# Hxyz-123/GoMatching

Hardware: AMD Instinct MI355X
Metric: frames/sec (whole node), 1280x720 clip, 100 queries/frame (higher is better)
Workload: dtype f32 (f16x3 split MFMA: 22-bit significand products, fp32 accumulate; parity tests at fp32 tolerances)

## Files before the change

gomatching_amd/csrc/msda.hip:

```cpp
#include <mutex>
#include <type_traits>
#include <vector>

#include "common.h"

namespace {

constexpr int HEADS = 8, CH = 32, LEVELS = 4;

__device__ __forceinline__ long xcd_contiguous_block(unsigned bid, unsigned nwg) {
    const unsigned q = nwg >> 3, r = nwg & 7, xcd = bid & 7;
    return (long)(xcd < r ? xcd * (q + 1) : r * (q + 1) + (xcd - r) * q) + (bid >> 3);
}

template <int POINTS>
__global__ __launch_bounds__(256) void msda_fwd_kernel(const float* __restrict__ value,
                                                       const int64_t* __restrict__ shapes,
                                                       const int64_t* __restrict__ lsi,
                                                       const float* __restrict__ loc,
                                                       const float* __restrict__ attw, float* __restrict__ out,
                                                       int B, int Lq, long v_bs, int v_rs) {
    const long q_global = xcd_contiguous_block(blockIdx.x, gridDim.x) * 4 + (threadIdx.x >> 6);
    if (q_global >= (long)B * Lq) return;
    const int lane = threadIdx.x & 63;
// ... 248 lines not shown
    const __amdgpu_buffer_rsrc_t rs = gom_buffer_rsrc(value + (size_t)b * v_bs, 0x7FFFFFFF);
    const unsigned mine = (unsigned)k * 16u;
    f32x4 acc = {0.f, 0.f, 0.f, 0.f};
#pragma unroll
    for (int i = 0; i < LP; ++i) {
        const int o = i >> 1, t = i & 1;
        const unsigned a1 = __builtin_bit_cast(unsigned, group8_read(__builtin_bit_cast(float, so1[t]), o)) + mine;
        const unsigned a2 = __builtin_bit_cast(unsigned, group8_read(__builtin_bit_cast(float, so2[t]), o)) + mine;
        const unsigned a3 = __builtin_bit_cast(unsigned, group8_read(__builtin_bit_cast(float, so3[t]), o)) + mine;
        const unsigned a4 = __builtin_bit_cast(unsigned, group8_read(__builtin_bit_cast(float, so4[t]), o)) + mine;
        const f32x4 v1 = __builtin_bit_cast(f32x4, __builtin_amdgcn_raw_buffer_load_b128(rs, (int)a1, 0, 0));
        const f32x4 v2 = __builtin_bit_cast(f32x4, __builtin_amdgcn_raw_buffer_load_b128(rs, (int)a2, 0, 0));
        const f32x4 v3 = __builtin_bit_cast(f32x4, __builtin_amdgcn_raw_buffer_load_b128(rs, (int)a3, 0, 0));
        const f32x4 v4 = __builtin_bit_cast(f32x4, __builtin_amdgcn_raw_buffer_load_b128(rs, (int)a4, 0, 0));
        const float w1 = group8_read(sw1[t], o), w2 = group8_read(sw2[t], o), w3 = group8_read(sw3[t], o), w4 = group8_read(sw4[t], o);
        msda_fma4(acc, w1, v1);
        msda_fma4(acc, w2, v2);
        msda_fma4(acc, w3, v3);
        msda_fma4(acc, w4, v4);
    }
    *reinterpret_cast<f32x4*>(out + (size_t)q_global * (HEADS * CH) + m * CH + k * 4) = acc;
}

template <int TY, int TX, int R, int CAP, int NB, int GLV = 0>
__global__ __launch_bounds__(256, 2) void msda_window_kernel(const float* __restrict__ value,
                                                             const int64_t* __restrict__ shapes,
                                                             const int64_t* __restrict__ lsi,
                                                             const float* __restrict__ raw, int ld_raw,
                                                             const float* __restrict__ ref, float* __restrict__ out,
                                                             int Lq, long v_bs, int v_rs, int tiles_y, int tiles_x, int ql,
                                                             unsigned* __restrict__ slow_groups) {
    constexpr int POINTS = 4, LP = LEVELS * POINTS, ITERS = (TY * TX) / 32;
    extern __shared__ __attribute__((aligned(16))) unsigned char win[];
    const int tid = threadIdx.x, lane = tid & 63;
    const int wave = __builtin_amdgcn_readfirstlane(tid >> 6);
    const int g = lane >> 3, k = lane & 7;
    const int m = (int)(blockIdx.x & 7u);
    unsigned tile = blockIdx.x >> 3;
    const int tx = (int)(tile % (unsigned)tiles_x);
    tile /= (unsigned)tiles_x;
    const int ty = (int)(tile % (unsigned)tiles_y);
    const int b = (int)(tile / (unsigned)tiles_y);
    const int l = k >> 1;

    int Hs[LEVELS], Ws[LEVELS];
    unsigned lv[LEVELS];
#pragma unroll
    for (int i = 0; i < LEVELS; ++i) {
        Hs[i] = (int)shapes[2 * i];
        Ws[i] = (int)shapes[2 * i + 1];
        lv[i] = (unsigned)lsi[i];
    }
    const int Hq = ql == 0 ? Hs[0] : ql == 1 ? Hs[1] : ql == 2 ? Hs[2] : Hs[3];
    const int Wq = ql == 0 ? Ws[0] : ql == 1 ? Ws[1] : ql == 2 ? Ws[2] : Ws[3];
    const long q0 = (long)b * Lq + (long)(ql == 0 ? lv[0] : ql == 1 ? lv[1] : ql == 2 ? lv[2] : lv[3]);
    const int y0t = ty * TY, x0t = tx * TX;
    const int y1t = min(y0t + TY, Hq) - 1, x1t = min(x0t + TX, Wq) - 1;
    const long qa = q0 + (long)y0t * Wq + x0t, qz = q0 + (long)y1t * Wq + x1t;
    const float rxa = ref[qa * 2], rya = ref[qa * 2 + 1], rxz = ref[qz * 2], ryz = ref[qz * 2 + 1];
    int wx0[LEVELS], wy0[LEVELS], wx1[LEVELS], wy1[LEVELS], wwd[LEVELS];
#pragma unroll
    for (int i = 0; i < LEVELS; ++i) {
        int ax = (int)floorf(fminf(rxa, rxz) * Ws[i] - 0.5f) - R, zx = (int)floorf(fmaxf(rxa, rxz) * Ws[i] - 0.5f) + R + 1;
        int ay = (int)floorf(fminf(rya, ryz) * Hs[i] - 0.5f) - R, zy = (int)floorf(fmaxf(rya, ryz) * Hs[i] - 0.5f) + R + 1;
        ax = max(ax, 0); ay = max(ay, 0); zx = min(zx, Ws[i] - 1); zy = min(zy, Hs[i] - 1);
        if (zx < ax) zx = ax;
        if (zy < ay) zy = ay;
        int w_ = zx - ax + 1, h_ = zy - ay + 1;
        if (w_ > CAP) { w_ = CAP; zx = ax + w_ - 1; }
        if (w_ * h_ > CAP) { h_ = CAP / w_; zy = ay + h_ - 1; }
        wx0[i] = ax; wy0[i] = ay; wx1[i] = zx; wy1[i] = zy; wwd[i] = w_;
    }
    const int H = l == 0 ? Hs[0] : l == 1 ? Hs[1] : l == 2 ? Hs[2] : Hs[3];
    const int W = l == 0 ? Ws[0] : l == 1 ? Ws[1] : l == 2 ? Ws[2] : Ws[3];
    const int mx0 = l == 0 ? wx0[0] : l == 1 ? wx0[1] : l == 2 ? wx0[2] : wx0[3];
    const int my0 = l == 0 ? wy0[0] : l == 1 ? wy0[1] : l == 2 ? wy0[2] : wy0[3];
    const int mx1 = l == 0 ? wx1[0] : l == 1 ? wx1[1] : l == 2 ? wx1[2] : wx1[3];
    const int my1 = l == 0 ? wy1[0] : l == 1 ? wy1[1] : l == 2 ? wy1[2] : wy1[3];
    const int mww = l == 0 ? wwd[0] : l == 1 ? wwd[1] : l == 2 ? wwd[2] : wwd[3];
    const unsigned lvl = l == 0 ? lv[0] : l == 1 ? lv[1] : l == 2 ? lv[2] : lv[3];
    const float Hf = (float)H, Wf = (float)W;
    const float rW = 1.f / Wf, rH = 1.f / Hf;

    const __amdgpu_buffer_rsrc_t rs = gom_buffer_rsrc(value + (size_t)b * v_bs, 0x7FFFFFFF);
    const unsigned mine = (unsigned)k * 16u;
    const unsigned head = (unsigned)(m * CH) * 4u;

    float sw1[ITERS][2], sw2[ITERS][2], sw3[ITERS][2], sw4[ITERS][2];
    unsigned pk[ITERS][2];
    unsigned go1[GLV ? ITERS : 1][2], go2[GLV ? ITERS : 1][2], go3[GLV ? ITERS : 1][2], go4[GLV ? ITERS : 1][2];
    f32x4 acc[ITERS];
    long qrow[ITERS];
    bool fast[ITERS], live[ITERS];
    f32x4 offs[ITERS];
    float lga[ITERS], lgb[ITERS], rxs[ITERS], rys[ITERS];
#pragma unroll
    for (int it = 0; it < ITERS; ++it) {
        const int j = (wave * ITERS + it) * 8 + g;
        const int jy = j / TX, jx = j - jy * TX;
        const int qy = y0t + jy, qx = x0t + jx;
        live[it] = qy <= y1t && qx <= x1t;
        const long q_global = q0 + (long)(live[it] ? qy : y0t) * Wq + (live[it] ? qx : x0t);
        qrow[it] = q_global;
        const float* op = raw + (size_t)q_global * ld_raw + m * (LP * 2) + 4 * k;
        const float* lp = raw + (size_t)q_global * ld_raw + HEADS * LP * 2 + m * LP + 2 * k;
        offs[it] = *reinterpret_cast<const f32x4*>(op);
        lga[it] = lp[0];
        lgb[it] = lp[1];
        rxs[it] = ref[q_global * 2];
        rys[it] = ref[q_global * 2 + 1];
    }
#define MSDA_GEOMETRY(IT, T, OFF4, RX, RY, E, INV_SUM, OK, SO)                                                    \
    {                                                                                                             \
        const float ox = (OFF4)[2 * (T)], oy = (OFF4)[2 * (T) + 1];                                               \
        float qx_ = ox * rW, qy_ = oy * rH;                                                                       \
        qx_ = fmaf(fmaf(-qx_, Wf, ox), rW, qx_);                                                                  \
        qy_ = fmaf(fmaf(-qy_, Hf, oy), rH, qy_);                                                                  \
        const float lx = (RX) + qx_, ly = (RY) + qy_;                                                             \
        const float w = (E) * (INV_SUM);                                                                          \
        const float h_im = ly * H - 0.5f, w_im = lx * W - 0.5f;                                                   \
        const bool inside = h_im > -1.f && w_im > -1.f && h_im < Hf && w_im < Wf;                                 \
        const float hf = floorf(h_im), wf = floorf(w_im);                                                         \
        const float lh = h_im - hf, lw = w_im - wf;                                                               \
        const float hh = 1.f - lh, hw = 1.f - lw;                                                                 \
        const int h_low = inside ? (int)hf : 0, w_low = inside ? (int)wf : 0;                                     \
        const bool y0 = h_low >= 0, y1 = h_low + 1 <= H - 1;                                                      \
        const bool x0 = w_low >= 0, x1 = w_low + 1 <= W - 1;                                                      \
        const int yc0 = y0 ? h_low : 0, yc1 = y1 ? h_low + 1 : H - 1;                                             \
        const int xc0 = x0 ? w_low : 0, xc1 = x1 ? w_low + 1 : W - 1;                                             \
        const unsigned r0 = lvl + (unsigned)(yc0 * W), r1 = lvl + (unsigned)(yc1 * W);                            \
        SO##1 = (r0 + xc0) * (unsigned)v_rs * 4u + head;                                                          \
        SO##2 = (r0 + xc1) * (unsigned)v_rs * 4u + head;                                                          \
        SO##3 = (r1 + xc0) * (unsigned)v_rs * 4u + head;                                                          \
        SO##4 = (r1 + xc1) * (unsigned)v_rs * 4u + head;                                                          \
        const float ww_ = inside ? w : 0.f;                                                                       \
        sw1[IT][T] = ((y0 && x0) ? hh * hw : 0.f) * ww_;                                                          \
        sw2[IT][T] = ((y0 && x1) ? hh * lw : 0.f) * ww_;                                                          \
        sw3[IT][T] = ((y1 && x0) ? lh * hw : 0.f) * ww_;                                                          \
        sw4[IT][T] = ((y1 && x1) ? lh * lw : 0.f) * ww_;                                                          \
         \
        OK = !inside || l < GLV || (yc0 >= my0 && yc1 <= my1 && xc0 >= mx0 && xc1 <= mx1);                        \
        const bool use = inside && OK;                          \
        const int ly0 = use ? yc0 - my0 : 0, lx0 = use ? xc0 - mx0 : 0;                                           \
        const unsigned la_ = (unsigned)((ly0 * mww + lx0) * 128);                                                 \
        pk[IT][T] = la_ | ((use && xc1 != xc0) ? (1u << 20) : 0u) | ((use && yc1 != yc0) ? (1u << 21) : 0u);      \
    }
    unsigned any_slow = 0;
#pragma unroll
    for (int it = 0; it < ITERS; ++it) {
        const float lg0 = lga[it], lg1 = lgb[it];
        float mx = fmaxf(lg0, lg1);
        mx = fmaxf(mx, __builtin_bit_cast(float, __builtin_amdgcn_ds_swizzle(__builtin_bit_cast(int, mx), 0x1F | (1 << 10))));
        mx = fmaxf(mx, __builtin_bit_cast(float, __builtin_amdgcn_ds_swizzle(__builtin_bit_cast(int, mx), 0x1F | (2 << 10))));
        mx = fmaxf(mx, __builtin_bit_cast(float, __builtin_amdgcn_ds_swizzle(__builtin_bit_cast(int, mx), 0x1F | (4 << 10))));
        const float e0 = expf(lg0 - mx), e1 = expf(lg1 - mx);
        float sum = 0.f;
#pragma unroll
        for (int o = 0; o < 8; ++o) {
            sum += group8_read(e0, o);
            sum += group8_read(e1, o);
        }
        const float inv_sum = 1.f / sum;
        bool ok0, ok1;
        unsigned sa1, sa2, sa3, sa4, sb1, sb2, sb3, sb4;
        MSDA_GEOMETRY(it, 0, offs[it], rxs[it], rys[it], e0, inv_sum, ok0, sa)
        MSDA_GEOMETRY(it, 1, offs[it], rxs[it], rys[it], e1, inv_sum, ok1, sb)
        if constexpr (GLV > 0) {
            go1[it][0] = sa1; go2[it][0] = sa2; go3[it][0] = sa3; go4[it][0] = sa4;
            go1[it][1] = sb1; go2[it][1] = sb2; go3[it][1] = sb3; go4[it][1] = sb4;
        }
        (void)sa1; (void)sa2; (void)sa3; (void)sa4; (void)sb1; (void)sb2; (void)sb3; (void)sb4;
        fast[it] = __builtin_amdgcn_ballot_w64(!(ok0 && ok1)) == 0;
        any_slow |= fast[it] ? 0u : 1u;
        acc[it] = f32x4{0.f, 0.f, 0.f, 0.f};
    }

    auto fill = [&](auto LEVC, unsigned char* buf) {
        constexpr int lev = decltype(LEVC)::value;
        const int ww_ = wwd[lev], n_lines = ww_ * (wy1[lev] - wy0[lev] + 1);
        const float inv_w = 1.f / (float)ww_;
        for (int base = wave * 8; base < n_lines; base += 32) {
            int line = base + g;
            if (line > n_lines - 1) line = n_lines - 1;
            int yy = (int)(((float)line + 0.5f) * inv_w);
            int xx = line - yy * ww_;
            if (xx < 0) { --yy; xx += ww_; }
            if (xx >= ww_) { ++yy; xx -= ww_; }
            const unsigned src = (lv[lev] + (unsigned)((wy0[lev] + yy) * Ws[lev] + wx0[lev] + xx)) * (unsigned)v_rs * 4u + head + mine;
            __builtin_amdgcn_raw_ptr_buffer_load_lds(rs, (__attribute__((address_space(3))) void*)(buf + (size_t)base * 128), 16,
                                                     (int)src, 0, 0, 0);
        }
    };
    auto bcast = [](float v, int owner) { return group8_read(v, owner); };
    auto level_samples = [&](auto LEVC, const unsigned char* buf) {
        constexpr int lev = decltype(LEVC)::value;
        typedef __attribute__((address_space(3))) f32x4 LdsF4;
        const unsigned mine_lds = mine + (unsigned)(size_t)buf;
        const unsigned row_bytes = (unsigned)wwd[lev] * 128u;
#pragma unroll
        for (int pnt = 0; pnt < POINTS; ++pnt) {
            const int i = lev * POINTS + pnt, o = i >> 1, t = i & 1;
#pragma unroll
            for (int half = 0; half < ITERS; half += NB) {
                bool any_fast = false;
#pragma unroll
                for (int u = 0; u < NB; ++u) any_fast = any_fast || fast[half + u];
                if (!any_fast) continue;
                unsigned word[NB];
                float w1[NB], w2[NB], w3[NB], w4[NB];
#pragma unroll
                for (int u = 0; u < NB; ++u) {
                    const int it = half + u;
                    asm volatile("" : "+v"(pk[it][t]), "+v"(sw1[it][t]), "+v"(sw2[it][t]), "+v"(sw3[it][t]), "+v"(sw4[it][t]));
                    word[u] = __builtin_bit_cast(unsigned, bcast(__builtin_bit_cast(float, pk[it][t]), o));
                    w1[u] = bcast(sw1[it][t], o);
                    w2[u] = bcast(sw2[it][t], o);
                    w3[u] = bcast(sw3[it][t], o);
                    w4[u] = bcast(sw4[it][t], o);
                }
                f32x4 v1[NB], v2[NB], v3[NB], v4[NB];
#pragma unroll
                for (int u = 0; u < NB; ++u) {
                    const unsigned a1 = (word[u] & 0xFFFFFu) + mine_lds;
                    const unsigned dx = (word[u] >> 20) & 1u, dy = (word[u] >> 21) & 1u;
                    unsigned a2 = a1 + dx * 128u, a3 = a1 + dy * row_bytes, a4 = a3 + dx * 128u;
                    asm volatile("" : "+v"(a2), "+v"(a3), "+v"(a4));
                    v1[u] = *reinterpret_cast<const LdsF4*>((size_t)a1);
                    v2[u] = *reinterpret_cast<const LdsF4*>((size_t)a2);
                    v3[u] = *reinterpret_cast<const LdsF4*>((size_t)a3);
                    v4[u] = *reinterpret_cast<const LdsF4*>((size_t)a4);
                }
#pragma unroll
                for (int u = 0; u < NB; ++u) {
                    msda_fma4(acc[half + u], w1[u], v1[u]);
                    msda_fma4(acc[half + u], w2[u], v2[u]);
                    msda_fma4(acc[half + u], w3[u], v3[u]);
                    msda_fma4(acc[half + u], w4[u], v4[u]);
                }
                __builtin_amdgcn_sched_barrier(0);
            }
        }
    };
#define MSDA_LEVEL_SINGLE(L)                                                                                      \
    {                                                                                                             \
        __syncthreads();                                                 \
        fill(std::integral_constant<int, L>{}, win);                                                              \
        asm volatile("s_waitcnt vmcnt(0)" ::: "memory");                                                          \
        __syncthreads();                                                                                          \
        level_samples(std::integral_constant<int, L>{}, win);                                                     \
    }
    auto level_gather = [&](auto LEVC) {
        constexpr int lev = decltype(LEVC)::value;
#pragma unroll
        for (int pnt = 0; pnt < POINTS; ++pnt) {
            const int i = lev * POINTS + pnt, o = i >> 1, t = i & 1;
#pragma unroll
            for (int half = 0; half < ITERS; half += NB) {
                bool any_fast = false;
#pragma unroll
                for (int u = 0; u < NB; ++u) any_fast = any_fast || fast[half + u];
                if (!any_fast) continue;
                unsigned a1[NB], a2[NB], a3[NB], a4[NB];
                float w1[NB], w2[NB], w3[NB], w4[NB];
#pragma unroll
                for (int u = 0; u < NB; ++u) {
                    const int it = half + u;
                    asm volatile("" : "+v"(go1[it][t]), "+v"(go2[it][t]), "+v"(go3[it][t]), "+v"(go4[it][t]));
                    asm volatile("" : "+v"(sw1[it][t]), "+v"(sw2[it][t]), "+v"(sw3[it][t]), "+v"(sw4[it][t]));
                    a1[u] = __builtin_bit_cast(unsigned, bcast(__builtin_bit_cast(float, go1[it][t]), o)) + mine;
                    a2[u] = __builtin_bit_cast(unsigned, bcast(__builtin_bit_cast(float, go2[it][t]), o)) + mine;
                    a3[u] = __builtin_bit_cast(unsigned, bcast(__builtin_bit_cast(float, go3[it][t]), o)) + mine;
                    a4[u] = __builtin_bit_cast(unsigned, bcast(__builtin_bit_cast(float, go4[it][t]), o)) + mine;
// ... 2 lines not shown
                    w3[u] = bcast(sw3[it][t], o);
                    w4[u] = bcast(sw4[it][t], o);
                }
                f32x4 v1[NB], v2[NB], v3[NB], v4[NB];
#pragma unroll
                for (int u = 0; u < NB; ++u) {
                    v1[u] = __builtin_bit_cast(f32x4, __builtin_amdgcn_raw_buffer_load_b128(rs, (int)a1[u], 0, 0));
                    v2[u] = __builtin_bit_cast(f32x4, __builtin_amdgcn_raw_buffer_load_b128(rs, (int)a2[u], 0, 0));
                    v3[u] = __builtin_bit_cast(f32x4, __builtin_amdgcn_raw_buffer_load_b128(rs, (int)a3[u], 0, 0));
                    v4[u] = __builtin_bit_cast(f32x4, __builtin_amdgcn_raw_buffer_load_b128(rs, (int)a4[u], 0, 0));
                }
#pragma unroll
                for (int u = 0; u < NB; ++u) {
                    msda_fma4(acc[half + u], w1[u], v1[u]);
                    msda_fma4(acc[half + u], w2[u], v2[u]);
                    msda_fma4(acc[half + u], w3[u], v3[u]);
                    msda_fma4(acc[half + u], w4[u], v4[u]);
                }
                __builtin_amdgcn_sched_barrier(0);
            }
        }
    };
    static_assert(GLV == 0 || GLV == 1, "only the finest level is ever gathered");
    if constexpr (GLV == 0) {
        MSDA_LEVEL_SINGLE(0)
    } else {
        fill(std::integral_constant<int, 1>{}, win);
        level_gather(std::integral_constant<int, 0>{});
    }
    if constexpr (GLV == 0) {
        MSDA_LEVEL_SINGLE(1)
    } else {
        asm volatile("s_waitcnt vmcnt(0)" ::: "memory");
        __syncthreads();
        level_samples(std::integral_constant<int, 1>{}, win);
    }
    MSDA_LEVEL_SINGLE(2) MSDA_LEVEL_SINGLE(3)
#undef MSDA_LEVEL_SINGLE
    if (any_slow) {
        if (slow_groups && lane == 0) {
            unsigned n_slow = 0;
#pragma unroll
            for (int it = 0; it < ITERS; ++it) n_slow += fast[it] ? 0u : 1u;
            atomicAdd(slow_groups, n_slow);
        }
#pragma unroll
        for (int it = 0; it < ITERS; ++it) {
            if (fast[it]) continue;
            const long q_global = qrow[it];
            const f32x4 off4 = *reinterpret_cast<const f32x4*>(raw + (size_t)q_global * ld_raw + m * (LP * 2) + 4 * k);
            const float* lp = raw + (size_t)q_global * ld_raw + HEADS * LP * 2 + m * LP + 2 * k;
            const float lg0 = lp[0], lg1 = lp[1];
            float mx = fmaxf(lg0, lg1);
            mx = fmaxf(mx, __builtin_bit_cast(float, __builtin_amdgcn_ds_swizzle(__builtin_bit_cast(int, mx), 0x1F | (1 << 10))));
            mx = fmaxf(mx, __builtin_bit_cast(float, __builtin_amdgcn_ds_swizzle(__builtin_bit_cast(int, mx), 0x1F | (2 << 10))));
            mx = fmaxf(mx, __builtin_bit_cast(float, __builtin_amdgcn_ds_swizzle(__builtin_bit_cast(int, mx), 0x1F | (4 << 10))));
            const float e0 = expf(lg0 - mx), e1 = expf(lg1 - mx);
            float sum = 0.f;
#pragma unroll
            for (int o = 0; o < 8; ++o) {
// ... 44 lines not shown
    return GOM_OK;
}

extern "C" int gom_msda_fused_forward(const float* raw, int ld_raw, const float* ref, const float* value,
                                      long value_batch_stride, int value_row_stride, const int64_t* spatial_shapes,
                                      const int64_t* level_start_index, float* output, int batch, int num_query,
                                      void* stream) {
    GOM_CHECK_ARG(raw && ref && value && spatial_shapes && level_start_index && output);
    GOM_CHECK_ARG(batch > 0 && num_query > 0 && ld_raw >= HEADS * LEVELS * 4 * 3 && (ld_raw % 4) == 0);
    GOM_CHECK_ARG(value_row_stride >= HEADS * CH && (value_row_stride % 4) == 0 && (value_batch_stride % 4) == 0);
    GOM_CHECK_ARG(((uintptr_t)raw % 16) == 0 && ((uintptr_t)value % 16) == 0);
    const long nq = (long)batch * num_query;
    if (g_msda_lanes && value_batch_stride > 0 && value_batch_stride < (1L << 29))
        hipLaunchKernelGGL((msda_fused_lanes_kernel<0>), dim3((unsigned)cdiv(nq, 4)), dim3(256), 0, (hipStream_t)stream,
                           value, spatial_shapes, level_start_index, raw, ld_raw, ref, output, batch, num_query,
                           value_batch_stride, value_row_stride, (const float*)nullptr, 0, num_query);
    else
        hipLaunchKernelGGL((msda_fused_kernel<4, 0>), dim3((unsigned)cdiv(nq, 4)), dim3(256), 0, (hipStream_t)stream, value,
                           spatial_shapes, level_start_index, raw, ld_raw, ref, output, batch, num_query,
                           value_batch_stride, value_row_stride, (const float*)nullptr);
    return gom_launch_status();
}

static int g_msda_window = 3;
static unsigned* g_msda_slow = nullptr;
extern "C" int gom_msda_set_window(int mask) {
    g_msda_window = mask < 0 ? 0 : (mask & 3);
    return GOM_OK;
}
extern "C" int gom_msda_window_count_fallbacks(unsigned int* device_counter) {
    g_msda_slow = device_counter;
    return GOM_OK;
}

extern "C" int gom_msda_fused_forward_encoder(const float* raw, int ld_raw, const float* ref, const float* value,
                                              long value_batch_stride, int value_row_stride, const int64_t* spatial_shapes,
                                              const int64_t* level_start_index, float* output, int batch, int num_query,
                                              int h0, int w0, int h1, int w1, void* stream) {
    GOM_CHECK_ARG(raw && ref && value && spatial_shapes && level_start_index && output);
    GOM_CHECK_ARG(batch > 0 && num_query > 0 && ld_raw >= HEADS * LEVELS * 4 * 3 && (ld_raw % 4) == 0);
    GOM_CHECK_ARG(value_row_stride >= HEADS * CH && (value_row_stride % 4) == 0 && (value_batch_stride % 4) == 0);
    GOM_CHECK_ARG(((uintptr_t)raw % 16) == 0 && ((uintptr_t)value % 16) == 0);
    GOM_CHECK_ARG(h0 > 0 && w0 > 0 && h1 >= 0 && w1 >= 0 && (long)h0 * w0 + (long)h1 * w1 <= num_query);
    constexpr int R = 5, CAP = 576;
    constexpr int TY0 = 8, TX0 = 16, TY1 = 8, TX1 = 16;
    const long n0 = (long)h0 * w0, n1 = (long)h1 * w1;
    const long wgs0 = (long)batch * cdiv(h0, TY0) * cdiv(w0, TX0) * 8;
    const long wgs1 = (long)batch * cdiv(h1, TY1) * cdiv(w1, TX1) * 8;
    if (!((g_msda_window & 1) && g_msda_lanes && value_batch_stride > 0 && value_batch_stride < (1L << 29) && wgs0 < (1L << 31) &&
          wgs1 < (1L << 31)))
        return gom_msda_fused_forward(raw, ld_raw, ref, value, value_batch_stride, value_row_stride, spatial_shapes,
                                      level_start_index, output, batch, num_query, stream);
    hipStream_t s = (hipStream_t)stream;
    {
        auto kern = msda_window_kernel<TY0, TX0, R, CAP, 4>;
        hipError_t e = hipFuncSetAttribute((const void*)kern, hipFuncAttributeMaxDynamicSharedMemorySize, CAP * 128);
        if (e != hipSuccess) return GOM_ERR_HIP_BASE + (int)e;
        hipLaunchKernelGGL(kern, dim3((unsigned)wgs0), dim3(256), CAP * 128, s, value, spatial_shapes, level_start_index, raw, ld_raw,
                           ref, output, num_query, value_batch_stride, value_row_stride, cdiv(h0, TY0), cdiv(w0, TX0), 0, g_msda_slow);
    }
    long done = n0;
    if ((g_msda_window & 2) && n1 > 0) {
        auto kern = msda_window_kernel<TY1, TX1, R, CAP, 4, 1>;
        hipError_t e = hipFuncSetAttribute((const void*)kern, hipFuncAttributeMaxDynamicSharedMemorySize, CAP * 128);
        if (e != hipSuccess) return GOM_ERR_HIP_BASE + (int)e;
        hipLaunchKernelGGL(kern, dim3((unsigned)wgs1), dim3(256), CAP * 128, s, value, spatial_shapes, level_start_index, raw, ld_raw,
                           ref, output, num_query, value_batch_stride, value_row_stride, cdiv(h1, TY1), cdiv(w1, TX1), 1, g_msda_slow);
        done += n1;
    }
    const long rest = num_query - done;
    if (rest > 0)
        hipLaunchKernelGGL((msda_fused_lanes_kernel<0>), dim3((unsigned)cdiv((long)batch * rest, 4)), dim3(256), 0, s, value,
                           spatial_shapes, level_start_index, raw, ld_raw, ref, output, batch, num_query, value_batch_stride,
                           value_row_stride, (const float*)nullptr, (int)done, (int)rest);
    return gom_launch_status();
}

extern "C" int gom_msda_fused_forward_vr(const float* raw, int ld_raw, const float* ref, const float* value,
                                         long value_batch_stride, int value_row_stride, const int64_t* spatial_shapes,
                                         const int64_t* level_start_index, const float* valid_ratios, float* output,
                                         int batch, int num_query, void* stream) {
    GOM_CHECK_ARG(raw && ref && value && spatial_shapes && level_start_index && valid_ratios && output);
    GOM_CHECK_ARG(batch > 0 && num_query > 0 && ld_raw >= HEADS * LEVELS * 4 * 3 && (ld_raw % 4) == 0);
    GOM_CHECK_ARG(value_row_stride >= HEADS * CH && (value_row_stride % 4) == 0 && (value_batch_stride % 4) == 0);
    GOM_CHECK_ARG(((uintptr_t)raw % 16) == 0 && ((uintptr_t)value % 16) == 0);
    const long nq = (long)batch * num_query;
    if (g_msda_lanes && value_batch_stride > 0 && value_batch_stride < (1L << 29))
        hipLaunchKernelGGL((msda_fused_lanes_kernel<1>), dim3((unsigned)cdiv(nq, 4)), dim3(256), 0, (hipStream_t)stream,
                           value, spatial_shapes, level_start_index, raw, ld_raw, ref, output, batch, num_query,
                           value_batch_stride, value_row_stride, valid_ratios, 0, num_query);
    else
        hipLaunchKernelGGL((msda_fused_kernel<4, 1>), dim3((unsigned)cdiv(nq, 4)), dim3(256), 0, (hipStream_t)stream, value,
                           spatial_shapes, level_start_index, raw, ld_raw, ref, output, batch, num_query,
                           value_batch_stride, value_row_stride, valid_ratios);
    return gom_launch_status();
}

extern "C" int gom_msda_fused_forward_vr_frames(const float* raw, int ld_raw, const float* ref, const float* value,
// ... 63 lines not shown
```

gomatching_amd/lib.py:

```python
import ctypes
import os
from ctypes import c_int, c_long, c_float, c_void_p

HERE = os.path.dirname(os.path.abspath(__file__))
LIB_PATH = os.environ.get("GOM_LIB_PATH") or os.path.join(HERE, "libgomatching_hip.so")

GOM_OK = 0
_ERR = {1: "GOM_ERR_INVALID_ARG (violated precondition)", 2: "GOM_ERR_UNSUPPORTED"}

P = c_void_p
I = c_int
L = c_long
F = c_float
D = ctypes.c_double
U = ctypes.c_uint
U64 = ctypes.c_ulonglong


class OptimTensor(ctypes.Structure):
    _fields_ = [("param", c_void_p), ("grad", c_void_p), ("exp_avg", c_void_p), ("exp_avg_sq", c_void_p),
                ("n", c_long), ("step", c_long), ("lr", ctypes.c_double), ("weight_decay", ctypes.c_double)]


SIGNATURES = {
    "gom_abi_version": (I, []),
    "gom_built_for_arch": (ctypes.c_char_p, []),
    "gom_ms_deform_attn_forward": (I, [P, P, P, P, P, P, I, I, I, I, I, I, I, P]),
    "gom_ms_deform_attn_forward_any": (I, [I, P, P, P, P, P, P, I, I, I, I, I, I, I, P]),
    "gom_ms_deform_attn_backward": (I, [I, P, P, P, P, P, P, P, P, P, I, I, I, I, I, I, I, P]),
    "gom_ms_deform_attn_forward_strided": (I, [P, L, I, P, P, P, P, P, I, I, P]),
    "gom_msda_set_lane_distributed": (I, [I]),
    "gom_msda_fused_forward": (I, [P, I, P, P, L, I, P, P, P, I, I, P]),
    "gom_msda_fused_forward_encoder": (I, [P, I, P, P, L, I, P, P, P, I, I, I, I, I, I, P]),
    "gom_msda_set_window": (I, [I]),
    "gom_msda_window_count_fallbacks": (I, [P]),
    "gom_msda_prepare": (I, [P, I, P, I, P, P, P, L, P]),
    "gom_gemm_f32": (I, [P, P, P, I, P, I, P, P, P, I, I, P, I, I, I, I, P]),
    "gom_gemm_splitk_workspace_bytes": (L, [I, I, I]),
    "gom_gemm_f32_splitk": (I, [P, P, I, P, I, P, P, P, I, I, P, I, I, I, I, P, L, P]),
    "gom_conv2d_nhwc_f32": (I, [P, P, P, P, P, I, P, I, I, I, I, I, I, I, I, I, P]),
    "gom_split_bf16x3": (I, [P, I, I, I, P, I, P]),
    "gom_gemm_f32_bf16x6": (I, [P, P, I, P, L, I, P, P, P, I, I, I, P, I, I, I, I, P]),
    "gom_conv2d_nhwc_f32_bf16x6": (I, [P, P, L, I, P, P, P, I, P, I, I, I, I, I, I, I, I, I, P]),
    "gom_gemm_small_f32": (I, [P, P, I, P, I, P, P, P, I, I, P, I, I, I, I, P]),
    "gom_conv_bf16x6_splits": (I, [I, I, I]),
    "gom_conv2d_nhwc_f32_bf16x6_splitk": (I, [P, P, L, I, P, P, P, I, P, I, I, I, I, I, I, I, I, I, P, L, I, P]),
    "gom_split_f16x2": (I, [P, I, I, I, P, I, P, P]),
    "gom_gemm_f32_f16x3": (I, [P, P, I, P, L, I, P, P, P, P, I, I, I, P, I, I, I, I, P, P]),
    "gom_gemm_f32_f16x3_rp": (I, [P, P, I, P, L, I, P, P, P, P, I, I, I, I, P, I, I, I, I, P, P]),
    "gom_conv2d_nhwc_f32_f16x3": (I, [P, P, L, I, P, P, P, P, I, P, I, I, I, I, I, I, I, I, I, P, L, I, P, P]),
    "gom_conv3x3_patch_supported": (I, [I, I]),
    "gom_conv3x3_patch_image_bytes": (L, [I, I]),
    "gom_conv3x3_patch_image": (I, [P, L, I, I, I, P, L, P]),
    "gom_conv3x3_patch_f32_f16x3": (I, [P, P, P, P, P, I, P, I, I, I, I, I, P, P]),
    "gom_bneck_image_bytes": (L, [I, I, I]),
    "gom_bneck_image": (I, [P, L, I, P, P, P, P, L, I, I, I, I, P, L, P]),
    "gom_bneck_f32": (I, [P, I, P, P, I, P, P, P, I, P, I, I, I, I, I, P, P]),
    "gom_bneck_sc_image_bytes": (L, [I, I, I, I, I]),
# ... 179 lines not shown
```

gomatching_amd/ops.py:

```python
import collections
import contextlib
import ctypes
import math

import numpy as np
import torch

from . import lib as _lib_mod
from .lib import check

_f32 = torch.float32


def _L():
    return _lib_mod.load()


_gemm_profile = None


_profile_scope = ""


@contextlib.contextmanager
# ... 989 lines not shown
    gv, gl, gw = torch.empty_like(value), torch.empty_like(sampling_loc), torch.empty_like(attn_weight)
    check(_L().gom_ms_deform_attn_backward(code, _p(value), _p(spatial_shapes), _p(level_start_index), _p(sampling_loc),
                                           _p(attn_weight), _p(grad_output), _p(gv), _p(gl), _p(gw), B, S, M, D, Lv, Lq, Pn,
                                           _stream()),
          "gom_ms_deform_attn_backward")
    return gv, gl, gw


def ms_deform_attn_forward_strided(value2d, batch_stride, shapes, lsi, loc, w, B, Lq):
    assert value2d.stride(1) == 1
    out = torch.empty((B * Lq, 256), dtype=_f32, device=value2d.device)
    check(_L().gom_ms_deform_attn_forward_strided(_p(value2d), batch_stride, value2d.stride(0), _p(shapes), _p(lsi),
                                                  _p(loc), _p(w), _p(out), B, Lq, _stream()),
          "gom_ms_deform_attn_forward_strided")
    return out


MSDA_LANES = _switch("MSDA_LANES")
_msda_lanes_set = [None]


MSDA_WINDOW = _switch("MSDA_WINDOW")
MSDA_WINDOW_L1 = _switch("MSDA_WINDOW_L1")
_msda_window_set = [None]


MSDA_WINDOW_POLICY = _switch("MSDA_WINDOW_POLICY")
MSDA_WINDOW_MAX_FALLBACK = 0.30


def msda_window_groups(encoder_hw0, B):
    h0, w0 = int(encoder_hw0[0]), int(encoder_hw0[1])
    n = -(-h0 // 8) * -(-w0 // 16) * 16
    if MSDA_WINDOW_L1 and len(encoder_hw0) >= 4:
        n += -(-int(encoder_hw0[2]) // 8) * -(-int(encoder_hw0[3]) // 16) * 16
    return B * 8 * n


def msda_fused(raw, ref, value2d, batch_stride, shapes, lsi, B, Lq, valid_ratios=None, encoder_hw0=None, fallback_counter=None,
               frame_valid_ratios=None):
    assert raw.stride(1) == 1 and value2d.stride(1) == 1
    _chk_f32(ref, valid_ratios)
    if frame_valid_ratios is not None:
        assert valid_ratios is None, "valid_ratios and frame_valid_ratios are exclusive"
        _chk_frame_desc(frame_valid_ratios, B, (shapes.shape[0], 2), _f32, "frame_valid_ratios")
    if _msda_lanes_set[0] != MSDA_LANES:
        _L().gom_msda_set_lane_distributed(1 if MSDA_LANES else 0)
        _msda_lanes_set[0] = MSDA_LANES
    out = torch.empty((B * Lq, 256), dtype=_f32, device=raw.device)
    S_rows = value2d.shape[0]
    with _timed(True, lambda: (2.0 * B * Lq * 8 * 16 * 4 * 32, 4.0 * (S_rows * 256 + B * Lq * (384 + 256)), "msda:%dx%d" % (B, Lq))):
        if frame_valid_ratios is not None:
            check(_L().gom_msda_fused_forward_vr_frames(_p(raw), raw.stride(0), _p(ref), _p(value2d), batch_stride,
                                                        value2d.stride(0), _p(shapes), _p(lsi), _p(frame_valid_ratios), _p(out),
                                                        B, Lq, _stream()), "gom_msda_fused_forward_vr_frames")
        elif valid_ratios is not None:
            check(_L().gom_msda_fused_forward_vr(_p(raw), raw.stride(0), _p(ref), _p(value2d), batch_stride,
                                                 value2d.stride(0), _p(shapes), _p(lsi), _p(valid_ratios), _p(out), B, Lq,
                                                 _stream()), "gom_msda_fused_forward_vr")
        elif encoder_hw0 is not None and MSDA_WINDOW and MSDA_LANES:
            mask = 3 if MSDA_WINDOW_L1 else 1
            if _msda_window_set[0] != mask:
                _L().gom_msda_set_window(mask)
                _msda_window_set[0] = mask
            h1, w1 = (int(encoder_hw0[2]), int(encoder_hw0[3])) if len(encoder_hw0) >= 4 else (0, 0)
            if fallback_counter is not None:
                fallback_counter.zero_()
                _L().gom_msda_window_count_fallbacks(_p(fallback_counter))
            try:
                check(_L().gom_msda_fused_forward_encoder(_p(raw), raw.stride(0), _p(ref), _p(value2d), batch_stride, value2d.stride(0),
                                                          _p(shapes), _p(lsi), _p(out), B, Lq, int(encoder_hw0[0]), int(encoder_hw0[1]),
                                                          h1, w1, _stream()), "gom_msda_fused_forward_encoder")
            finally:
                if fallback_counter is not None:
                    _L().gom_msda_window_count_fallbacks(None)
        else:
            check(_L().gom_msda_fused_forward(_p(raw), raw.stride(0), _p(ref), _p(value2d), batch_stride, value2d.stride(0),
                                              _p(shapes), _p(lsi), _p(out), B, Lq, _stream()), "gom_msda_fused_forward")
    return out


def msda_prepare(raw, ref, spatial_shapes, ref_levels=1):
    _chk_f32(ref)
    Q = raw.shape[0]
# ... 1051 lines not shown
```

include/gomatching_hip.h:

```cpp
#ifndef GOMATCHING_HIP_H_
#define GOMATCHING_HIP_H_

#include <stdint.h>

#ifdef __cplusplus
extern "C" {
#endif

#define GOM_OK 0
#define GOM_ERR_INVALID_ARG 1
#define GOM_ERR_UNSUPPORTED 2
#define GOM_ERR_HIP_BASE 1000

#define GOM_DTYPE_F32 0
#define GOM_DTYPE_F64 1

#define GOM_ABI_VERSION 1
int gom_abi_version(void);
const char* gom_built_for_arch(void);

int gom_ms_deform_attn_forward(const float* value, const int64_t* spatial_shapes, const int64_t* level_start_index,
                               const float* sampling_loc, const float* attn_weight, float* output, int batch,
                               int spatial_size, int num_heads, int channels, int num_levels, int num_query,
                               int num_point, void* stream);

int gom_ms_deform_attn_forward_any(int dtype, const void* value, const int64_t* spatial_shapes,
                                   const int64_t* level_start_index, const void* sampling_loc, const void* attn_weight,
                                   void* output, int batch, int spatial_size, int num_heads, int channels, int num_levels,
                                   int num_query, int num_point, void* stream);

int gom_ms_deform_attn_backward(int dtype, const void* value, const int64_t* spatial_shapes,
                                const int64_t* level_start_index, const void* sampling_loc, const void* attn_weight,
                                const void* grad_output, void* grad_value, void* grad_sampling_loc, void* grad_attn_weight,
                                int batch, int spatial_size, int num_heads, int channels, int num_levels, int num_query,
                                int num_point, void* stream);

int gom_ms_deform_attn_forward_strided(const float* value, long value_batch_stride, int value_row_stride,
                                       const int64_t* spatial_shapes, const int64_t* level_start_index,
                                       const float* sampling_loc, const float* attn_weight, float* output, int batch,
                                       int num_query, void* stream);

int gom_msda_set_lane_distributed(int on);
int gom_msda_fused_forward(const float* raw, int ld_raw, const float* ref, const float* value, long value_batch_stride,
                           int value_row_stride, const int64_t* spatial_shapes, const int64_t* level_start_index,
                           float* output, int batch, int num_query, void* stream);
int gom_msda_set_window(int mask);
int gom_msda_window_count_fallbacks(unsigned int* device_counter);
int gom_msda_fused_forward_encoder(const float* raw, int ld_raw, const float* ref, const float* value, long value_batch_stride,
                                   int value_row_stride, const int64_t* spatial_shapes, const int64_t* level_start_index,
                                   float* output, int batch, int num_query, int h0, int w0, int h1, int w1, void* stream);

int gom_msda_prepare(const float* raw, int ld_raw, const float* ref, int ref_levels, const int64_t* spatial_shapes,
                     float* sampling_loc, float* attn_weight, long num_query_total, void* stream);

int gom_gemm_f32(const float* A, const float* A2, const int* a_rows, int lda, const float* W, int ldw,
                 const float* scale, const float* shift, const float* R, int ldr, int relu, float* C, int ldc, int M,
                 int N, int K, void* stream);

long gom_gemm_splitk_workspace_bytes(int M, int N, int K);
int gom_gemm_f32_splitk(const float* A, const int* a_rows, int lda, const float* W, int ldw, const float* scale,
                        const float* shift, const float* R, int ldr, int relu, float* C, int ldc, int M, int N, int K,
                        void* workspace, long workspace_bytes, void* stream);

int gom_conv2d_nhwc_f32(const float* X, const float* Wt, const float* scale, const float* shift, const float* R,
                        int relu, float* Y, int B, int H, int Wd, int Cin, int Cout, int KH, int KW, int stride,
                        int pad, void* stream);

int gom_gemm_small_f32(const float* A, const int* a_rows, int lda, const float* W, int ldw, const float* scale,
                       const float* shift, const float* R, int ldr, int relu, float* C, int ldc, int M, int N, int K,
                       void* stream);
// ... 428 lines not shown
```

Measured before the change: 305.9.

## Overlap MSDA window LDS fills with sampling by packing levels into split regions

Adds an overlap schedule (OVL) to the windowed MSDA encoder kernel. The LDS window is partitioned so two pyramid levels can sit in it at once: level 0 is filled before geometry runs, and later levels are filled while earlier ones are being sampled. This hides the global-to-LDS fill latency behind compute instead of serialising a fill-wait-sample step per level. The cost is smaller per-level window caps, which can push more queries onto the slow fallback path. It also adds hand-written ds_read and lgkmcnt waits, gated by a new mask bit and a Python switch, plus a host helper that reports the window plan.

```diff
diff --git a/gomatching_amd/csrc/msda.hip b/gomatching_amd/csrc/msda.hip
--- a/gomatching_amd/csrc/msda.hip
+++ b/gomatching_amd/csrc/msda.hip
@@ -294,7 +294,36 @@
     *reinterpret_cast<f32x4*>(out + (size_t)q_global * (HEADS * CH) + m * CH + k * 4) = acc;
 }
 
-template <int TY, int TX, int R, int CAP, int NB, int GLV = 0>
+template <int R, int CAP>
+__host__ __device__ __forceinline__ void msda_window_plan(const int (&Hs)[LEVELS], const int (&Ws)[LEVELS], float rxa, float rya,
+                                                          float rxz, float ryz, int glv, int schedule, int (&wx0)[LEVELS],
+                                                          int (&wy0)[LEVELS], int (&wx1)[LEVELS], int (&wy1)[LEVELS],
+                                                          int (&wwd)[LEVELS], int (&wst)[LEVELS]) {
+    static_assert(CAP % 8 == 0 && CAP >= 16, "regions are whole groups of 8 lines");
+    const int first = glv == 0 ? 1 : 2;
+    int split = 0;
+#pragma unroll
+    for (int i = 0; i < LEVELS; ++i) {
+        int ax = (int)floorf(fminf(rxa, rxz) * Ws[i] - 0.5f) - R, zx = (int)floorf(fmaxf(rxa, rxz) * Ws[i] - 0.5f) + R + 1;
+        int ay = (int)floorf(fminf(rya, ryz) * Hs[i] - 0.5f) - R, zy = (int)floorf(fmaxf(rya, ryz) * Hs[i] - 0.5f) + R + 1;
+        ax = ax > 0 ? ax : 0; ay = ay > 0 ? ay : 0; zx = zx < Ws[i] - 1 ? zx : Ws[i] - 1; zy = zy < Hs[i] - 1 ? zy : Hs[i] - 1;
+        if (zx < ax) zx = ax;
+        if (zy < ay) zy = ay;
+        int start = 0, cap = CAP;
+        if (schedule == 1) {
+            if (i == first) cap = CAP - 8;
+            if (i == first + 1) { start = split; cap = CAP - split; }
+            if (glv == 0 && i == 3) cap = split;
+        }
+        int w_ = zx - ax + 1, h_ = zy - ay + 1;
+        if (w_ > cap) { w_ = cap; zx = ax + w_ - 1; }
+        if (w_ * h_ > cap) { h_ = cap / w_; zy = ay + h_ - 1; }
+        if (i == first) split = (w_ * h_ + 7) & ~7;
+        wx0[i] = ax; wy0[i] = ay; wx1[i] = zx; wy1[i] = zy; wwd[i] = w_; wst[i] = start;
+    }
+}
+
+template <int TY, int TX, int R, int CAP, int NB, int GLV = 0, int OVL = 0>
 __global__ __launch_bounds__(256, 2) void msda_window_kernel(const float* __restrict__ value,
                                                              const int64_t* __restrict__ shapes,
                                                              const int64_t* __restrict__ lsi,
@@ -330,19 +359,8 @@
     const int y1t = min(y0t + TY, Hq) - 1, x1t = min(x0t + TX, Wq) - 1;
     const long qa = q0 + (long)y0t * Wq + x0t, qz = q0 + (long)y1t * Wq + x1t;
     const float rxa = ref[qa * 2], rya = ref[qa * 2 + 1], rxz = ref[qz * 2], ryz = ref[qz * 2 + 1];
-    int wx0[LEVELS], wy0[LEVELS], wx1[LEVELS], wy1[LEVELS], wwd[LEVELS];
-#pragma unroll
-    for (int i = 0; i < LEVELS; ++i) {
-        int ax = (int)floorf(fminf(rxa, rxz) * Ws[i] - 0.5f) - R, zx = (int)floorf(fmaxf(rxa, rxz) * Ws[i] - 0.5f) + R + 1;
-        int ay = (int)floorf(fminf(rya, ryz) * Hs[i] - 0.5f) - R, zy = (int)floorf(fmaxf(rya, ryz) * Hs[i] - 0.5f) + R + 1;
-        ax = max(ax, 0); ay = max(ay, 0); zx = min(zx, Ws[i] - 1); zy = min(zy, Hs[i] - 1);
-        if (zx < ax) zx = ax;
-        if (zy < ay) zy = ay;
-        int w_ = zx - ax + 1, h_ = zy - ay + 1;
-        if (w_ > CAP) { w_ = CAP; zx = ax + w_ - 1; }
-        if (w_ * h_ > CAP) { h_ = CAP / w_; zy = ay + h_ - 1; }
-        wx0[i] = ax; wy0[i] = ay; wx1[i] = zx; wy1[i] = zy; wwd[i] = w_;
-    }
+    int wx0[LEVELS], wy0[LEVELS], wx1[LEVELS], wy1[LEVELS], wwd[LEVELS], wst[LEVELS];
+    msda_window_plan<R, CAP>(Hs, Ws, rxa, rya, rxz, ryz, GLV, OVL, wx0, wy0, wx1, wy1, wwd, wst);
     const int H = l == 0 ? Hs[0] : l == 1 ? Hs[1] : l == 2 ? Hs[2] : Hs[3];
     const int W = l == 0 ? Ws[0] : l == 1 ? Ws[1] : l == 2 ? Ws[2] : Ws[3];
     const int mx0 = l == 0 ? wx0[0] : l == 1 ? wx0[1] : l == 2 ? wx0[2] : wx0[3];
@@ -350,6 +368,7 @@
     const int mx1 = l == 0 ? wx1[0] : l == 1 ? wx1[1] : l == 2 ? wx1[2] : wx1[3];
     const int my1 = l == 0 ? wy1[0] : l == 1 ? wy1[1] : l == 2 ? wy1[2] : wy1[3];
     const int mww = l == 0 ? wwd[0] : l == 1 ? wwd[1] : l == 2 ? wwd[2] : wwd[3];
+    const int mst = l == 0 ? wst[0] : l == 1 ? wst[1] : l == 2 ? wst[2] : wst[3];
     const unsigned lvl = l == 0 ? lv[0] : l == 1 ? lv[1] : l == 2 ? lv[2] : lv[3];
     const float Hf = (float)H, Wf = (float)W;
     const float rW = 1.f / Wf, rH = 1.f / Hf;
@@ -381,6 +400,28 @@
         lgb[it] = lp[1];
         rxs[it] = ref[q_global * 2];
         rys[it] = ref[q_global * 2 + 1];
+    }
+    auto fill = [&](auto LEVC) {
+        constexpr int lev = decltype(LEVC)::value;
+        unsigned char* buf = win + (size_t)wst[lev] * 128;
+        const int ww_ = wwd[lev], n_lines = ww_ * (wy1[lev] - wy0[lev] + 1);
+        const float inv_w = 1.f / (float)ww_;
+        for (int base = wave * 8; base < n_lines; base += 32) {
+            int line = base + g;
+            if (line > n_lines - 1) line = n_lines - 1;
+            int yy = (int)(((float)line + 0.5f) * inv_w);
+            int xx = line - yy * ww_;
+            if (xx < 0) { --yy; xx += ww_; }
+            if (xx >= ww_) { ++yy; xx -= ww_; }
+            const unsigned src = (lv[lev] + (unsigned)((wy0[lev] + yy) * Ws[lev] + wx0[lev] + xx)) * (unsigned)v_rs * 4u + head + mine;
+            __builtin_amdgcn_raw_ptr_buffer_load_lds(rs, (__attribute__((address_space(3))) void*)(buf + (size_t)base * 128), 16,
+                                                     (int)src, 0, 0, 0);
+        }
+    };
+    if constexpr (OVL != 0) {
+#pragma unroll
+        for (int it = 0; it < ITERS; ++it) asm volatile("" : "+v"(offs[it]), "+v"(lga[it]), "+v"(lgb[it]), "+v"(rxs[it]), "+v"(rys[it]));
+        fill(std::integral_constant<int, GLV>{});
     }
 #define MSDA_GEOMETRY(IT, T, OFF4, RX, RY, E, INV_SUM, OK, SO)                                                    \
     {                                                                                                             \
@@ -414,7 +455,7 @@
         OK = !inside || l < GLV || (yc0 >= my0 && yc1 <= my1 && xc0 >= mx0 && xc1 <= mx1);                        \
         const bool use = inside && OK;                          \
         const int ly0 = use ? yc0 - my0 : 0, lx0 = use ? xc0 - mx0 : 0;                                           \
-        const unsigned la_ = (unsigned)((ly0 * mww + lx0) * 128);                                                 \
+        const unsigned la_ = (unsigned)((mst + ly0 * mww + lx0) * 128);                                           \
         pk[IT][T] = la_ | ((use && xc1 != xc0) ? (1u << 20) : 0u) | ((use && yc1 != yc0) ? (1u << 21) : 0u);      \
     }
     unsigned any_slow = 0;
@@ -447,25 +488,10 @@
         acc[it] = f32x4{0.f, 0.f, 0.f, 0.f};
     }
 
-    auto fill = [&](auto LEVC, unsigned char* buf) {
+    auto bcast = [](float v, int owner) { return group8_read(v, owner); };
+    auto level_samples = [&](auto LEVC, const unsigned char* buf, auto UNDERC) {
         constexpr int lev = decltype(LEVC)::value;
-        const int ww_ = wwd[lev], n_lines = ww_ * (wy1[lev] - wy0[lev] + 1);
-        const float inv_w = 1.f / (float)ww_;
-        for (int base = wave * 8; base < n_lines; base += 32) {
-            int line = base + g;
-            if (line > n_lines - 1) line = n_lines - 1;
-            int yy = (int)(((float)line + 0.5f) * inv_w);
-            int xx = line - yy * ww_;
-            if (xx < 0) { --yy; xx += ww_; }
-            if (xx >= ww_) { ++yy; xx -= ww_; }
-            const unsigned src = (lv[lev] + (unsigned)((wy0[lev] + yy) * Ws[lev] + wx0[lev] + xx)) * (unsigned)v_rs * 4u + head + mine;
-            __builtin_amdgcn_raw_ptr_buffer_load_lds(rs, (__attribute__((address_space(3))) void*)(buf + (size_t)base * 128), 16,
-                                                     (int)src, 0, 0, 0);
-        }
-    };
-    auto bcast = [](float v, int owner) { return group8_read(v, owner); };
-    auto level_samples = [&](auto LEVC, const unsigned char* buf) {
-        constexpr int lev = decltype(LEVC)::value;
+        constexpr bool under = decltype(UNDERC)::value;
         typedef __attribute__((address_space(3))) f32x4 LdsF4;
         const unsigned mine_lds = mine + (unsigned)(size_t)buf;
         const unsigned row_bytes = (unsigned)wwd[lev] * 128u;
@@ -497,10 +523,23 @@
                     const unsigned dx = (word[u] >> 20) & 1u, dy = (word[u] >> 21) & 1u;
                     unsigned a2 = a1 + dx * 128u, a3 = a1 + dy * row_bytes, a4 = a3 + dx * 128u;
                     asm volatile("" : "+v"(a2), "+v"(a3), "+v"(a4));
-                    v1[u] = *reinterpret_cast<const LdsF4*>((size_t)a1);
-                    v2[u] = *reinterpret_cast<const LdsF4*>((size_t)a2);
-                    v3[u] = *reinterpret_cast<const LdsF4*>((size_t)a3);
-                    v4[u] = *reinterpret_cast<const LdsF4*>((size_t)a4);
+                    if constexpr (under) {
+                        asm volatile("ds_read_b128 %0, %1" : "=&v"(v1[u]) : "v"(a1));
+                        asm volatile("ds_read_b128 %0, %1" : "=&v"(v2[u]) : "v"(a2));
+                        asm volatile("ds_read_b128 %0, %1" : "=&v"(v3[u]) : "v"(a3));
+                        asm volatile("ds_read_b128 %0, %1" : "=&v"(v4[u]) : "v"(a4));
+                    } else {
+                        v1[u] = *reinterpret_cast<const LdsF4*>((size_t)a1);
+                        v2[u] = *reinterpret_cast<const LdsF4*>((size_t)a2);
+                        v3[u] = *reinterpret_cast<const LdsF4*>((size_t)a3);
+                        v4[u] = *reinterpret_cast<const LdsF4*>((size_t)a4);
+                    }
+                }
+                if constexpr (under) {
+                    static_assert(4 * (NB - 1) < 16, "lgkmcnt counts to 15");
+#pragma unroll
+                    for (int u = 0; u < NB; ++u)
+                        asm volatile("s_waitcnt lgkmcnt(%4)" : "+v"(v1[u]), "+v"(v2[u]), "+v"(v3[u]), "+v"(v4[u]) : "n"(4 * (NB - 1 - u)));
                 }
 #pragma unroll
                 for (int u = 0; u < NB; ++u) {
@@ -516,10 +555,10 @@
 #define MSDA_LEVEL_SINGLE(L)                                                                                      \
     {                                                                                                             \
         __syncthreads();                                                 \
-        fill(std::integral_constant<int, L>{}, win);                                                              \
+        fill(std::integral_constant<int, L>{});                                                                   \
         asm volatile("s_waitcnt vmcnt(0)" ::: "memory");                                                          \
         __syncthreads();                                                                                          \
-        level_samples(std::integral_constant<int, L>{}, win);                                                     \
+        level_samples(std::integral_constant<int, L>{}, win, std::false_type{});                                  \
     }
     auto level_gather = [&](auto LEVC) {
         constexpr int lev = decltype(LEVC)::value;
@@ -568,20 +607,50 @@
         }
     };
     static_assert(GLV == 0 || GLV == 1, "only the finest level is ever gathered");
-    if constexpr (GLV == 0) {
-        MSDA_LEVEL_SINGLE(0)
+    static_assert(OVL == 0 || OVL == 1, "two fill schedules");
+#define MSDA_LANDED()                                                                                             \
+    {                                                                                                             \
+        asm volatile("s_waitcnt vmcnt(0)" ::: "memory");                                                          \
+        __syncthreads();                                                                                          \
+    }
+    if constexpr (OVL == 0 && GLV == 0) {
+        MSDA_LEVEL_SINGLE(0) MSDA_LEVEL_SINGLE(1) MSDA_LEVEL_SINGLE(2) MSDA_LEVEL_SINGLE(3)
+    } else if constexpr (OVL == 0) {
+        fill(std::integral_constant<int, 1>{});
+        level_gather(std::integral_constant<int, 0>{});
+        MSDA_LANDED()
+        level_samples(std::integral_constant<int, 1>{}, win, std::false_type{});
+        MSDA_LEVEL_SINGLE(2) MSDA_LEVEL_SINGLE(3)
+    } else if constexpr (GLV == 0) {
+#pragma unroll
+        for (int it = 0; it < ITERS; ++it)
+            asm volatile("" ::"v"(pk[it][0]), "v"(pk[it][1]), "v"(sw1[it][0]), "v"(sw2[it][0]), "v"(sw3[it][0]), "v"(sw4[it][0]),
+                         "v"(sw1[it][1]), "v"(sw2[it][1]), "v"(sw3[it][1]), "v"(sw4[it][1]));
+        __builtin_amdgcn_sched_barrier(0);
+        MSDA_LANDED()
+        level_samples(std::integral_constant<int, 0>{}, win, std::false_type{});
+        __syncthreads();
+        fill(std::integral_constant<int, 1>{});
+        fill(std::integral_constant<int, 2>{});
+        MSDA_LANDED()
+        level_samples(std::integral_constant<int, 1>{}, win, std::false_type{});
+        __syncthreads();
+        fill(std::integral_constant<int, 3>{});
+        level_samples(std::integral_constant<int, 2>{}, win, std::true_type{});
+        MSDA_LANDED()
+        level_samples(std::integral_constant<int, 3>{}, win, std::false_type{});
     } else {
-        fill(std::integral_constant<int, 1>{}, win);
         level_gather(std::integral_constant<int, 0>{});
-    }
-    if constexpr (GLV == 0) {
-        MSDA_LEVEL_SINGLE(1)
-    } else {
-        asm volatile("s_waitcnt vmcnt(0)" ::: "memory");
+        MSDA_LANDED()
+        level_samples(std::integral_constant<int, 1>{}, win, std::false_type{});
         __syncthreads();
-        level_samples(std::integral_constant<int, 1>{}, win);
-    }
-    MSDA_LEVEL_SINGLE(2) MSDA_LEVEL_SINGLE(3)
+        fill(std::integral_constant<int, 2>{});
+        fill(std::integral_constant<int, 3>{});
+        MSDA_LANDED()
+        level_samples(std::integral_constant<int, 2>{}, win, std::false_type{});
+        level_samples(std::integral_constant<int, 3>{}, win, std::false_type{});
+    }
+#undef MSDA_LANDED
 #undef MSDA_LEVEL_SINGLE
     if (any_slow) {
         if (slow_groups && lane == 0) {
@@ -672,10 +741,10 @@
     return gom_launch_status();
 }
 
-static int g_msda_window = 3;
+static int g_msda_window = 7;
 static unsigned* g_msda_slow = nullptr;
 extern "C" int gom_msda_set_window(int mask) {
-    g_msda_window = mask < 0 ? 0 : (mask & 3);
+    g_msda_window = mask < 0 ? 0 : (mask & 7);
     return GOM_OK;
 }
 extern "C" int gom_msda_window_count_fallbacks(unsigned int* device_counter) {
@@ -702,8 +771,9 @@
         return gom_msda_fused_forward(raw, ld_raw, ref, value, value_batch_stride, value_row_stride, spatial_shapes,
                                       level_start_index, output, batch, num_query, stream);
     hipStream_t s = (hipStream_t)stream;
+    const bool ovl = (g_msda_window & 4) != 0;
     {
-        auto kern = msda_window_kernel<TY0, TX0, R, CAP, 4>;
+        auto kern = ovl ? msda_window_kernel<TY0, TX0, R, CAP, 4, 0, 1> : msda_window_kernel<TY0, TX0, R, CAP, 4, 0, 0>;
         hipError_t e = hipFuncSetAttribute((const void*)kern, hipFuncAttributeMaxDynamicSharedMemorySize, CAP * 128);
         if (e != hipSuccess) return GOM_ERR_HIP_BASE + (int)e;
         hipLaunchKernelGGL(kern, dim3((unsigned)wgs0), dim3(256), CAP * 128, s, value, spatial_shapes, level_start_index, raw, ld_raw,
@@ -711,7 +781,7 @@
     }
     long done = n0;
     if ((g_msda_window & 2) && n1 > 0) {
-        auto kern = msda_window_kernel<TY1, TX1, R, CAP, 4, 1>;
+        auto kern = ovl ? msda_window_kernel<TY1, TX1, R, CAP, 4, 1, 1> : msda_window_kernel<TY1, TX1, R, CAP, 4, 1, 0>;
         hipError_t e = hipFuncSetAttribute((const void*)kern, hipFuncAttributeMaxDynamicSharedMemorySize, CAP * 128);
         if (e != hipSuccess) return GOM_ERR_HIP_BASE + (int)e;
         hipLaunchKernelGGL(kern, dim3((unsigned)wgs1), dim3(256), CAP * 128, s, value, spatial_shapes, level_start_index, raw, ld_raw,
@@ -724,6 +794,29 @@
                            spatial_shapes, level_start_index, raw, ld_raw, ref, output, batch, num_query, value_batch_stride,
                            value_row_stride, (const float*)nullptr, (int)done, (int)rest);
     return gom_launch_status();
+}
+
+extern "C" int gom_msda_window_plan(const int64_t* spatial_shapes, int tile_level, const float* ref_first, const float* ref_last,
+                                    int schedule, int* plan, int* cap_lines) {
+    GOM_CHECK_ARG(spatial_shapes && ref_first && ref_last && plan && cap_lines);
+    GOM_CHECK_ARG((tile_level == 0 || tile_level == 1) && (schedule == 0 || schedule == 1));
+    constexpr int R = 5, CAP = 576;
+    int Hs[LEVELS], Ws[LEVELS], wx0[LEVELS], wy0[LEVELS], wx1[LEVELS], wy1[LEVELS], wwd[LEVELS], wst[LEVELS];
+    for (int i = 0; i < LEVELS; ++i) {
+        GOM_CHECK_ARG(spatial_shapes[2 * i] > 0 && spatial_shapes[2 * i + 1] > 0);
+        Hs[i] = (int)spatial_shapes[2 * i];
+        Ws[i] = (int)spatial_shapes[2 * i + 1];
+    }
+    msda_window_plan<R, CAP>(Hs, Ws, ref_first[0], ref_first[1], ref_last[0], ref_last[1], tile_level, schedule, wx0, wy0, wx1, wy1,
+                             wwd, wst);
+    for (int i = 0; i < LEVELS; ++i) {
+        const bool gathered = i < tile_level;
+        plan[3 * i] = gathered ? 0 : wst[i];
+        plan[3 * i + 1] = gathered ? 0 : wwd[i];
+        plan[3 * i + 2] = gathered ? 0 : wy1[i] - wy0[i] + 1;
+    }
+    *cap_lines = CAP;
+    return GOM_OK;
 }
 
 extern "C" int gom_msda_fused_forward_vr(const float* raw, int ld_raw, const float* ref, const float* value,
diff --git a/gomatching_amd/lib.py b/gomatching_amd/lib.py
--- a/gomatching_amd/lib.py
+++ b/gomatching_amd/lib.py
@@ -34,6 +34,7 @@
     "gom_msda_fused_forward_encoder": (I, [P, I, P, P, L, I, P, P, P, I, I, I, I, I, I, P]),
     "gom_msda_set_window": (I, [I]),
     "gom_msda_window_count_fallbacks": (I, [P]),
+    "gom_msda_window_plan": (I, [P, I, P, P, I, P, P]),
     "gom_msda_prepare": (I, [P, I, P, I, P, P, P, L, P]),
     "gom_gemm_f32": (I, [P, P, P, I, P, I, P, P, P, I, I, P, I, I, I, I, P]),
     "gom_gemm_splitk_workspace_bytes": (L, [I, I, I]),
diff --git a/gomatching_amd/ops.py b/gomatching_amd/ops.py
--- a/gomatching_amd/ops.py
+++ b/gomatching_amd/ops.py
@@ -1035,6 +1035,7 @@
 
 MSDA_WINDOW = _switch("MSDA_WINDOW")
 MSDA_WINDOW_L1 = _switch("MSDA_WINDOW_L1")
+MSDA_WINDOW_OVERLAP = _switch("MSDA_WINDOW_OVERLAP")
 _msda_window_set = [None]
 
 
@@ -1072,7 +1073,7 @@
                                                  value2d.stride(0), _p(shapes), _p(lsi), _p(valid_ratios), _p(out), B, Lq,
                                                  _stream()), "gom_msda_fused_forward_vr")
         elif encoder_hw0 is not None and MSDA_WINDOW and MSDA_LANES:
-            mask = 3 if MSDA_WINDOW_L1 else 1
+            mask = (3 if MSDA_WINDOW_L1 else 1) | (4 if MSDA_WINDOW_OVERLAP else 0)
             if _msda_window_set[0] != mask:
                 _L().gom_msda_set_window(mask)
                 _msda_window_set[0] = mask
diff --git a/include/gomatching_hip.h b/include/gomatching_hip.h
--- a/include/gomatching_hip.h
+++ b/include/gomatching_hip.h
@@ -46,6 +46,8 @@
                            float* output, int batch, int num_query, void* stream);
 int gom_msda_set_window(int mask);
 int gom_msda_window_count_fallbacks(unsigned int* device_counter);
+int gom_msda_window_plan(const int64_t* spatial_shapes, int tile_level, const float* ref_first, const float* ref_last, int schedule,
+                         int* plan, int* cap_lines);
 int gom_msda_fused_forward_encoder(const float* raw, int ld_raw, const float* ref, const float* value, long value_batch_stride,
                                    int value_row_stride, const int64_t* spatial_shapes, const int64_t* level_start_index,
                                    float* output, int batch, int num_query, int h0, int w0, int h1, int w1, void* stream);
```

Result: faster. 309.4 (median of 6 runs) (+1.2%).
